# fbcotter/pytorch_wavelets

Measured on NVIDIA B200. Metric: Mpixels/sec DWT J=3 db4 + DTCWT J=3 fwd, higher is better.
Workload: dtype f32

## Files before the change

pytorch_wavelets_b200/csrc/b200wave.cu:

```cuda
#include <cuda_runtime.h>
#include <stdio.h>

#include "launch_params.h"
#include "fast_api.h"

namespace b200w {
constexpr int NT = 256;
extern __shared__ __align__(16) float g_smem[];

__global__ void __launch_bounds__(NT) k_afb2d_tile(const __grid_constant__ AfbParams p) { afb2d_tile<NT>(p, blockIdx.x, g_smem); }
__global__ void __launch_bounds__(NT) k_sfb2d_tile(const __grid_constant__ SfbParams p) { sfb2d_tile<NT>(p, blockIdx.x, g_smem); }
__global__ void __launch_bounds__(NT) k_fwd_j1_tile(const __grid_constant__ DtParams p) { fwd_j1_tile<NT, false>(p, blockIdx.x, g_smem); }
__global__ void __launch_bounds__(NT) k_scat_j1_tile(const __grid_constant__ DtParams p) { fwd_j1_tile<NT, true>(p, blockIdx.x, g_smem); }
__global__ void __launch_bounds__(NT) k_fwd_j2plus_tile(const __grid_constant__ DtParams p) { fwd_j2plus_tile<NT>(p, blockIdx.x, g_smem); }
__global__ void __launch_bounds__(NT) k_inv_j1_tile(const __grid_constant__ DtParams p) { inv_j1_tile<NT>(p, blockIdx.x, g_smem); }
__global__ void __launch_bounds__(NT) k_inv_j2plus_tile(const __grid_constant__ DtParams p) { inv_j2plus_tile<NT>(p, blockIdx.x, g_smem); }

}

using namespace b200w;

namespace {

thread_local char g_last_cuda_error[256] = "";

int check_launch() {
  cudaError_t e = cudaGetLastError();
  if (e != cudaSuccess) {
    snprintf(g_last_cuda_error, sizeof(g_last_cuda_error), "%s: %s", cudaGetErrorName(e), cudaGetErrorString(e));
    return B200W_ECUDA;
  }
  return B200W_OK;
}

template <class K>
int set_smem(K kernel, size_t bytes) {
  if (bytes > 48 * 1024) {
    if (bytes > 227 * 1024) return B200W_EFILTER;
    cudaError_t e = cudaFuncSetAttribute(kernel, cudaFuncAttributeMaxDynamicSharedMemorySize, (int)bytes);
    if (e != cudaSuccess) {
      snprintf(g_last_cuda_error, sizeof(g_last_cuda_error), "%s: %s", cudaGetErrorName(e), cudaGetErrorString(e));
      return B200W_ECUDA;
    }
  }
  return 0;
}

template <class K, class P>
int launch_tile(K kernel, const P& p, long long blocks, int smem_floats, void* stream) {
  if (blocks == 0) return B200W_OK;
  const size_t bytes = (size_t)smem_floats * sizeof(float);
  int rc = set_smem(kernel, bytes);
  if (rc) return rc;
  kernel<<<(unsigned)blocks, NT, bytes, (cudaStream_t)stream>>>(p);
  return check_launch();
}

}

namespace {

static int dwt_afb2d_impl(const float* x, long long x_plane_stride, int x_pitch, float* ll, long long ll_plane_stride,
                    int ll_pitch, float* highs, int planes, int H, int W, const float* fw_lo, const float* fw_hi,
                    int Lw, const float* fh_lo, const float* fh_hi, int Lh, int mode, void* stream, bool generic) {
  AfbParams p;
  int rc = build_afb(p, x, x_plane_stride, x_pitch, ll, ll_plane_stride, ll_pitch, highs, planes, H, W, fw_lo,
                     fw_hi, Lw, fh_lo, fh_hi, Lh, mode);
  if (rc) return rc;
  rc = generic ? fast::kNoFastPath : fast::try_launch_afb(p, (cudaStream_t)stream);
  if (rc != fast::kNoFastPath) return rc ? rc : check_launch();
  return launch_tile(k_afb2d_tile, p, (long long)planes * p.tiles_x * p.tiles_y, afb_smem_floats(Lw, Lh), stream);
}

static int dwt_sfb2d_impl(const float* ll, long long ll_plane_stride, int ll_pitch, const float* highs, float* y,
                    long long y_plane_stride, int y_pitch, int planes, int Hc, int Wc, int Ho, int Wo,
                    const float* gh_lo, const float* gh_hi, int Lh, const float* gw_lo, const float* gw_hi, int Lw,
                    int mode, void* stream, bool generic) {
  SfbParams p;
  int rc = build_sfb(p, ll, ll_plane_stride, ll_pitch, highs, y, y_plane_stride, y_pitch, planes, Hc, Wc, Ho, Wo,
                     gh_lo, gh_hi, Lh, gw_lo, gw_hi, Lw, mode);
  if (rc) return rc;
  rc = generic ? fast::kNoFastPath : fast::try_launch_sfb(p, (cudaStream_t)stream);
  if (rc != fast::kNoFastPath) return rc ? rc : check_launch();
  return launch_tile(k_sfb2d_tile, p, (long long)planes * p.tiles_x * p.tiles_y, sfb_smem_floats(Lh, Lw), stream);
}

static int dtcwt_fwd_j1_impl(const float* x, long long x_plane_stride, int x_pitch, float* ll, long long ll_plane_stride,
                       int ll_pitch, float* highs, const long long hs[6], int N, int C, int H, int W,
                       const float* h0, int L0, const float* h1, int L1, int mode, void* stream, bool generic) {
  DtParams p;
  int rc = build_fwd_j1(p, x, x_plane_stride, x_pitch, ll, ll_plane_stride, ll_pitch, highs, hs, N, C, H, W, h0, L0,
                        h1, L1, mode);
  if (rc) return rc;
  rc = generic ? fast::kNoFastPath : fast::try_launch_fwd_j1(p, (cudaStream_t)stream);
  if (rc != fast::kNoFastPath) return rc ? rc : check_launch();
  return launch_tile(k_fwd_j1_tile, p, (long long)N * C * p.tiles_x * p.tiles_y, fwdj1_smem_floats(L0, L1), stream);
}

static int dtcwt_fwd_j2plus_impl(const float* x, long long x_plane_stride, int x_pitch, float* ll,
                           long long ll_plane_stride, int ll_pitch, float* highs, const long long hs[6], int N,
                           int C, int H, int W, const float* h0a, const float* h1a, const float* h0b,
                           const float* h1b, int m, void* stream, bool generic) {
  DtParams p;
  int rc = build_fwd_j2plus(p, x, x_plane_stride, x_pitch, ll, ll_plane_stride, ll_pitch, highs, hs, N, C, H, W,
                            h0a, h1a, h0b, h1b, m);
  if (rc) return rc;
  rc = generic ? fast::kNoFastPath : fast::try_launch_fwd_j2plus(p, (cudaStream_t)stream);
  if (rc != fast::kNoFastPath) return rc ? rc : check_launch();
  return launch_tile(k_fwd_j2plus_tile, p, (long long)N * C * p.tiles_x * p.tiles_y, fwdj2_smem_floats(m), stream);
}

static int dtcwt_inv_j1_impl(const float* ll, long long ll_plane_stride, int ll_pitch, const float* highs,
                       const long long hs[6], float* y, long long y_plane_stride, int y_pitch, int N, int C, int H,
                       int W, const float* g0, int L0, const float* g1, int L1, int mode, void* stream, bool generic) {
  DtParams p;
  int rc = build_inv_j1(p, ll, ll_plane_stride, ll_pitch, highs, hs, y, y_plane_stride, y_pitch, N, C, H, W, g0, L0,
                        g1, L1, mode);
  if (rc) return rc;
  rc = generic ? fast::kNoFastPath : fast::try_launch_inv_j1(p, (cudaStream_t)stream);
  if (rc != fast::kNoFastPath) return rc ? rc : check_launch();
  return launch_tile(k_inv_j1_tile, p, (long long)N * C * p.tiles_x * p.tiles_y, invj1_smem_floats(L0, L1), stream);
}

static int dtcwt_inv_j2plus_impl(const float* ll, long long ll_plane_stride, int ll_pitch, const float* highs,
                           const long long hs[6], float* y, long long y_plane_stride, int y_pitch, int N, int C,
                           int H, int W, const float* g0a, const float* g1a, const float* g0b, const float* g1b,
                           int m, void* stream, bool generic) {
  DtParams p;
  int rc = build_inv_j2plus(p, ll, ll_plane_stride, ll_pitch, highs, hs, y, y_plane_stride, y_pitch, N, C, H, W,
                            g0a, g1a, g0b, g1b, m);
  if (rc) return rc;
  rc = generic ? fast::kNoFastPath : fast::try_launch_inv_j2plus(p, (cudaStream_t)stream);
  if (rc != fast::kNoFastPath) return rc ? rc : check_launch();
  return launch_tile(k_inv_j2plus_tile, p, (long long)N * C * p.tiles_x * p.tiles_y, invj2_smem_floats(m), stream);
}

static int scat_j1_impl(const float* x, float* z, float* dre_dr, float* dim_dr, int N, int C, int H, int W,
                  const float* h0, int L0, const float* h1, int L1, int mode, float magbias, void* stream, bool generic) {
  DtParams p;
  int rc = build_scat_j1(p, x, z, dre_dr, dim_dr, N, C, H, W, h0, L0, h1, L1, mode, magbias);
  if (rc) return rc;
  rc = generic ? fast::kNoFastPath : fast::try_launch_scat_j1(p, (cudaStream_t)stream);
  if (rc != fast::kNoFastPath) return rc ? rc : check_launch();
  return launch_tile(k_scat_j1_tile, p, (long long)N * C * p.tiles_x * p.tiles_y, fwdj1_smem_floats(L0, L1), stream);
}

}

extern "C" {

int b200w_version(void) { return B200W_VERSION; }

const char* b200w_strerror(int code) {
  switch (code) {
    case B200W_OK: return "ok";
    case B200W_EMODE: return "Unkown pad type";
    case B200W_ESIZE: return "bad tensor size";
    case B200W_EARG: return "bad argument";
    case B200W_EFILTER: return "unsupported filter length";
    case B200W_ECUDA: return "CUDA error";
    case B200W_ENOTIMPL: return "not implemented";
    default: return "unknown error";
  }
}

const char* b200w_last_cuda_error(void) { return g_last_cuda_error; }

int b200w_dwt_coeff_len(int n, int flen, int mode) { return coeff_len(n, flen, mode); }
int b200w_dwt_rec_len(int k, int flen, int mode) { return rec_len(k, flen, mode); }

int b200w_dwt_afb2d(const float* x, long long x_plane_stride, int x_pitch, float* ll, long long ll_plane_stride,
                    int ll_pitch, float* highs, int planes, int H, int W, const float* fw_lo, const float* fw_hi,
                    int Lw, const float* fh_lo, const float* fh_hi, int Lh, int mode, void* stream) {
  return dwt_afb2d_impl(x, x_plane_stride, x_pitch, ll, ll_plane_stride, ll_pitch, highs, planes, H, W, fw_lo, fw_hi, Lw, fh_lo, fh_hi, Lh, mode, stream, false);
}
int b200w_dwt_afb2d_generic(const float* x, long long x_plane_stride, int x_pitch, float* ll, long long ll_plane_stride,
                    int ll_pitch, float* highs, int planes, int H, int W, const float* fw_lo, const float* fw_hi,
                    int Lw, const float* fh_lo, const float* fh_hi, int Lh, int mode, void* stream) {
  return dwt_afb2d_impl(x, x_plane_stride, x_pitch, ll, ll_plane_stride, ll_pitch, highs, planes, H, W, fw_lo, fw_hi, Lw, fh_lo, fh_hi, Lh, mode, stream, true);
}

int b200w_dwt_sfb2d(const float* ll, long long ll_plane_stride, int ll_pitch, const float* highs, float* y,
                    long long y_plane_stride, int y_pitch, int planes, int Hc, int Wc, int Ho, int Wo,
                    const float* gh_lo, const float* gh_hi, int Lh, const float* gw_lo, const float* gw_hi, int Lw,
                    int mode, void* stream) {
  return dwt_sfb2d_impl(ll, ll_plane_stride, ll_pitch, highs, y, y_plane_stride, y_pitch, planes, Hc, Wc, Ho, Wo, gh_lo, gh_hi, Lh, gw_lo, gw_hi, Lw, mode, stream, false);
}
int b200w_dwt_sfb2d_generic(const float* ll, long long ll_plane_stride, int ll_pitch, const float* highs, float* y,
                    long long y_plane_stride, int y_pitch, int planes, int Hc, int Wc, int Ho, int Wo,
                    const float* gh_lo, const float* gh_hi, int Lh, const float* gw_lo, const float* gw_hi, int Lw,
                    int mode, void* stream) {
  return dwt_sfb2d_impl(ll, ll_plane_stride, ll_pitch, highs, y, y_plane_stride, y_pitch, planes, Hc, Wc, Ho, Wo, gh_lo, gh_hi, Lh, gw_lo, gw_hi, Lw, mode, stream, true);
}

int b200w_dtcwt_fwd_j1(const float* x, long long x_plane_stride, int x_pitch, float* ll, long long ll_plane_stride,
                       int ll_pitch, float* highs, const long long hs[6], int N, int C, int H, int W,
                       const float* h0, int L0, const float* h1, int L1, int mode, void* stream) {
  return dtcwt_fwd_j1_impl(x, x_plane_stride, x_pitch, ll, ll_plane_stride, ll_pitch, highs, hs, N, C, H, W, h0, L0, h1, L1, mode, stream, false);
}
int b200w_dtcwt_fwd_j1_generic(const float* x, long long x_plane_stride, int x_pitch, float* ll, long long ll_plane_stride,
                       int ll_pitch, float* highs, const long long hs[6], int N, int C, int H, int W,
                       const float* h0, int L0, const float* h1, int L1, int mode, void* stream) {
  return dtcwt_fwd_j1_impl(x, x_plane_stride, x_pitch, ll, ll_plane_stride, ll_pitch, highs, hs, N, C, H, W, h0, L0, h1, L1, mode, stream, true);
}

int b200w_dtcwt_fwd_j2plus(const float* x, long long x_plane_stride, int x_pitch, float* ll,
                           long long ll_plane_stride, int ll_pitch, float* highs, const long long hs[6], int N,
                           int C, int H, int W, const float* h0a, const float* h1a, const float* h0b,
                           const float* h1b, int m, void* stream) {
  return dtcwt_fwd_j2plus_impl(x, x_plane_stride, x_pitch, ll, ll_plane_stride, ll_pitch, highs, hs, N, C, H, W, h0a, h1a, h0b, h1b, m, stream, false);
}
int b200w_dtcwt_fwd_j2plus_generic(const float* x, long long x_plane_stride, int x_pitch, float* ll,
                           long long ll_plane_stride, int ll_pitch, float* highs, const long long hs[6], int N,
                           int C, int H, int W, const float* h0a, const float* h1a, const float* h0b,
                           const float* h1b, int m, void* stream) {
  return dtcwt_fwd_j2plus_impl(x, x_plane_stride, x_pitch, ll, ll_plane_stride, ll_pitch, highs, hs, N, C, H, W, h0a, h1a, h0b, h1b, m, stream, true);
}

int b200w_dtcwt_inv_j1(const float* ll, long long ll_plane_stride, int ll_pitch, const float* highs,
                       const long long hs[6], float* y, long long y_plane_stride, int y_pitch, int N, int C, int H,
                       int W, const float* g0, int L0, const float* g1, int L1, int mode, void* stream) {
  return dtcwt_inv_j1_impl(ll, ll_plane_stride, ll_pitch, highs, hs, y, y_plane_stride, y_pitch, N, C, H, W, g0, L0, g1, L1, mode, stream, false);
}
int b200w_dtcwt_inv_j1_generic(const float* ll, long long ll_plane_stride, int ll_pitch, const float* highs,
                       const long long hs[6], float* y, long long y_plane_stride, int y_pitch, int N, int C, int H,
                       int W, const float* g0, int L0, const float* g1, int L1, int mode, void* stream) {
  return dtcwt_inv_j1_impl(ll, ll_plane_stride, ll_pitch, highs, hs, y, y_plane_stride, y_pitch, N, C, H, W, g0, L0, g1, L1, mode, stream, true);
}

int b200w_dtcwt_inv_j2plus(const float* ll, long long ll_plane_stride, int ll_pitch, const float* highs,
                           const long long hs[6], float* y, long long y_plane_stride, int y_pitch, int N, int C,
                           int H, int W, const float* g0a, const float* g1a, const float* g0b, const float* g1b,
                           int m, void* stream) {
  return dtcwt_inv_j2plus_impl(ll, ll_plane_stride, ll_pitch, highs, hs, y, y_plane_stride, y_pitch, N, C, H, W, g0a, g1a, g0b, g1b, m, stream, false);
}
int b200w_dtcwt_inv_j2plus_generic(const float* ll, long long ll_plane_stride, int ll_pitch, const float* highs,
                           const long long hs[6], float* y, long long y_plane_stride, int y_pitch, int N, int C,
                           int H, int W, const float* g0a, const float* g1a, const float* g0b, const float* g1b,
                           int m, void* stream) {
  return dtcwt_inv_j2plus_impl(ll, ll_plane_stride, ll_pitch, highs, hs, y, y_plane_stride, y_pitch, N, C, H, W, g0a, g1a, g0b, g1b, m, stream, true);
}


static long long align256(long long n) { return (n + 255) / 256 * 256; }

static void dwt_ws_layout(int planes, int H, int W, int J, int Lw, int Lh, int mode, long long bytes[2]) {
  bytes[0] = bytes[1] = 0;
  int h = H, w = W;
  for (int j = 0; j + 1 < J; ++j) {
    h = coeff_len(h, Lh, mode); w = coeff_len(w, Lw, mode);
    if (h < 1 || w < 1) break;
    const long long need = align256(4LL * planes * h * ((w + 31) / 32 * 32));
    if (need > bytes[j & 1]) bytes[j & 1] = need;
  }
}

enum DwtPolicy { kLevels = 0, kPyramidFirst = 1, kPyramidAll = 2 };

#ifndef B200W_PYR_FUSE_ALL_MIN_WIDTH
#define B200W_PYR_FUSE_ALL_MIN_WIDTH 1024
#endif

static DwtPolicy dwt_policy(PyrParams& pp, const float* x, long long xps, int xpitch, int planes, int H, int W, int J,
                            int Lw, int Lh, int mode, bool generic) {
  if (generic || Lw != Lh) return kLevels;
  const bool wide = (W >= B200W_PYR_FUSE_ALL_MIN_WIDTH);
  if ((J == 1 || wide) && fast::plan_dwt_pyramid(pp, x, xps, xpitch, planes, H, W, J, Lw, mode, 0) == 0)
    return kPyramidAll;
  if (J >= 2) {
    const int wo = coeff_len(W, Lw, mode);
    if (wo > 0 && fast::plan_dwt_pyramid(pp, x, xps, xpitch, planes, H, W, 1, Lw, mode, (wo + 31) / 32 * 32) == 0)
      return kPyramidFirst;
  }
  return kLevels;
}

long long b200w_dwt_forward_workspace(const float* x, long long x_plane_stride, int x_pitch, int planes, int H, int W,
                                      int J, int Lw, int Lh, int mode) {
  if (!dwt_mode_ok(mode)) return B200W_EMODE;
  if (planes < 0 || H < 1 || W < 1 || J < 1) return B200W_ESIZE;
  if (Lw < 2 || Lh < 2 || Lw > kMaxTaps || Lh > kMaxTaps) return B200W_EFILTER;
  PyrParams pp;
  if (dwt_policy(pp, x, x_plane_stride, x_pitch, planes, H, W, J, Lw, Lh, mode, false) == kPyramidAll) return 0;
  long long b[2];
  dwt_ws_layout(planes, H, W, J, Lw, Lh, mode, b);
  return b[0] + b[1];
}

static void pyr_set_taps(PyrParams& pp, const float* fw_lo, const float* fw_hi, const float* fh_lo, const float* fh_hi,
                         int L) {
  for (int i = 0; i < kPyrMaxTaps; ++i) {
    const bool on = i < L;
    pp.fw[2 * i] = on ? fw_lo[i] : 0.f; pp.fw[2 * i + 1] = on ? fw_hi[i] : 0.f;
    pp.fh_lo[i] = on ? fh_lo[i] : 0.f; pp.fh_hi[i] = on ? fh_hi[i] : 0.f;
  }
}

static int dwt_forward_impl(const float* x, long long x_plane_stride, int x_pitch, int planes, int H, int W, int J,
                            float* yl, float* const* highs, const float* fw_lo, const float* fw_hi, int Lw,
                            const float* fh_lo, const float* fh_hi, int Lh, int mode, void* workspace,
                            long long workspace_bytes, void* stream, bool generic) {
  if (!dwt_mode_ok(mode)) return B200W_EMODE;
  if (!x || !yl || !highs || !fw_lo || !fw_hi || !fh_lo || !fh_hi) return B200W_EARG;
  if (planes < 0 || H < 1 || W < 1 || J < 1) return B200W_ESIZE;
  if (Lw < 2 || Lh < 2) return B200W_EFILTER;
  for (int j = 0; j < J; ++j)
    if (!highs[j]) return B200W_EARG;
  PyrParams pp;
  DwtPolicy pol = dwt_policy(pp, x, x_plane_stride, x_pitch, planes, H, W, J, Lw, Lh, mode, generic);
  if (pol == kPyramidAll) {
    pyr_set_taps(pp, fw_lo, fw_hi, fh_lo, fh_hi, Lw);
    pp.yl = yl;
    for (int j = 0; j < kPyrMaxLevels; ++j) pp.highs[j] = (j < J) ? highs[j] : nullptr;
    const int rc = fast::launch_dwt_pyramid(pp, (cudaStream_t)stream);
    if (rc != fast::kNoFastPath) return rc ? rc : check_launch();
    pol = kLevels;
  }
  long long wb[2];
  dwt_ws_layout(planes, H, W, J, Lw, Lh, mode, wb);
  if (wb[0] + wb[1] > 0 && (!workspace || workspace_bytes < wb[0] + wb[1])) return B200W_EARG;
  float* buf[2] = {static_cast<float*>(workspace), reinterpret_cast<float*>(static_cast<char*>(workspace) + wb[0])};
  const float* src = x;
  long long sps = x_plane_stride;
  int spitch = x_pitch, h = H, w = W;
  for (int j = 0; j < J; ++j) {
    const int ho = coeff_len(h, Lh, mode), wo = coeff_len(w, Lw, mode);
    if (ho < 1 || wo < 1) return B200W_ESIZE;
    const bool last = (j == J - 1);
    const int wp = last ? wo : (wo + 31) / 32 * 32;
    float* ll = last ? yl : buf[j & 1];
    int rc = fast::kNoFastPath;
    if (j == 0 && pol == kPyramidFirst) {
      pyr_set_taps(pp, fw_lo, fw_hi, fh_lo, fh_hi, Lw);
      pp.yl = ll;
      for (int i = 0; i < kPyrMaxLevels; ++i) pp.highs[i] = (i == 0) ? highs[0] : nullptr;
      rc = fast::launch_dwt_pyramid(pp, (cudaStream_t)stream);
      if (rc == 0) rc = check_launch();
    }
    if (rc == fast::kNoFastPath)
      rc = dwt_afb2d_impl(src, sps, spitch, ll, (long long)ho * wp, wp, highs[j], planes, h, w, fw_lo, fw_hi, Lw, fh_lo,
                          fh_hi, Lh, mode, stream, generic);
    if (rc) return rc;
    src = ll; sps = (long long)ho * wp; spitch = wp; h = ho; w = wo;
  }
  return B200W_OK;
}

int b200w_dwt_forward(const float* x, long long x_plane_stride, int x_pitch, int planes, int H, int W, int J, float* yl,
                      float* const* highs, const float* fw_lo, const float* fw_hi, int Lw, const float* fh_lo,
                      const float* fh_hi, int Lh, int mode, void* workspace, long long workspace_bytes, void* stream) {
  return dwt_forward_impl(x, x_plane_stride, x_pitch, planes, H, W, J, yl, highs, fw_lo, fw_hi, Lw, fh_lo, fh_hi, Lh,
                          mode, workspace, workspace_bytes, stream, false);
}
int b200w_dwt_forward_generic(const float* x, long long x_plane_stride, int x_pitch, int planes, int H, int W, int J,
                              float* yl, float* const* highs, const float* fw_lo, const float* fw_hi, int Lw,
                              const float* fh_lo, const float* fh_hi, int Lh, int mode, void* workspace,
                              long long workspace_bytes, void* stream) {
  return dwt_forward_impl(x, x_plane_stride, x_pitch, planes, H, W, J, yl, highs, fw_lo, fw_hi, Lw, fh_lo, fh_hi, Lh,
                          mode, workspace, workspace_bytes, stream, true);
}

int b200w_scat_j1(const float* x, float* z, float* dre_dr, float* dim_dr, int N, int C, int H, int W,
                  const float* h0, int L0, const float* h1, int L1, int mode, float magbias, void* stream) {
  return scat_j1_impl(x, z, dre_dr, dim_dr, N, C, H, W, h0, L0, h1, L1, mode, magbias, stream, false);
}
int b200w_scat_j1_generic(const float* x, float* z, float* dre_dr, float* dim_dr, int N, int C, int H, int W,
                  const float* h0, int L0, const float* h1, int L1, int mode, float magbias, void* stream) {
  return scat_j1_impl(x, z, dre_dr, dim_dr, N, C, H, W, h0, L0, h1, L1, mode, magbias, stream, true);
}

}
```

pytorch_wavelets_b200/csrc/dwt_pyramid.cuh:

```cuda
#pragma once
#include "pyramid_plan.h"
#include "stream_common.cuh"

namespace b200w {
namespace fast {

#ifdef B200W_PYR_PROF
__device__ unsigned long long g_pyr_prof[64];
#define PYR_T0() const long long pyr_t0_ = clock64()
#define PYR_ACC(k) prof[k] += (unsigned long long)(clock64() - pyr_t0_)
#define PYR_DECL() unsigned long long prof[8] = {0, 0, 0, 0, 0, 0, 0, 0}; const long long pyr_life_ = clock64()
#define PYR_FLUSH(role, lane)                                                                              \
  do {                                                                                                     \
    prof[7] = (unsigned long long)(clock64() - pyr_life_);                                                 \
    if ((lane) == 0)                                                                                       \
      for (int k_ = 0; k_ < 8; ++k_) atomicAdd(&g_pyr_prof[8 * (role) + k_], prof[k_]);                    \
  } while (0)
#else
#define PYR_T0() do {} while (0)
#define PYR_ACC(k) do {} while (0)
#define PYR_DECL() do {} while (0)
#define PYR_FLUSH(role, lane) do {} while (0)
#endif

constexpr int kPyrNSlotC = B200W_PYR_NSLOT;

template <int L>
struct PyrCfg {
  static constexpr int NC = kPyrNC;
  static constexpr int PL = L - 2;
  static constexpr int PRO = PL / 2;
  static constexpr int UNR = L / 2;
  static constexpr int HS = pyr_hs(L);
  static constexpr int RS = 2 * HS;
  static constexpr int HALO = pyr_halo(L);
  static constexpr int NX = 2 * NC + PL;
  static_assert(HS >= 4 && HS % 2 == 0 && HS % UNR == 0, "stage = whole window periods, even");
};

__device__ __forceinline__ void mbar_arrive(unsigned bar) {
  asm volatile("mbarrier.arrive.shared::cta.b64 _, [%0];\n" ::"r"(bar) : "memory");
}
__device__ __forceinline__ bool mbar_test(unsigned bar, unsigned parity) {
  unsigned ok;
  asm volatile(
      "{\n.reg .pred p;\n"
      "mbarrier.test_wait.parity.shared::cta.b64 p, [%1], %2;\n"
      "selp.u32 %0, 1, 0, p;\n}\n"
      : "=r"(ok)
      : "r"(bar), "r"(parity)
      : "memory");
  return ok != 0;
}
__device__ __forceinline__ void mbar_wait_relaxed(unsigned bar, unsigned parity) {
  while (!mbar_test(bar, parity)) __nanosleep(200);
}
__device__ __forceinline__ void bulk_store_s2g(float* gdst, unsigned ssrc, unsigned bytes) {
  asm volatile("cp.async.bulk.global.shared::cta.bulk_group [%0], [%1], %2;\n" ::"l"(gdst), "r"(ssrc), "r"(bytes) : "memory");
}
__device__ __forceinline__ void bulk_commit() { asm volatile("cp.async.bulk.commit_group;\n" ::: "memory"); }
template <int N>
__device__ __forceinline__ void bulk_wait_read() { asm volatile("cp.async.bulk.wait_group.read %0;\n" ::"n"(N) : "memory"); }
template <int N>
__device__ __forceinline__ void bulk_wait() { asm volatile("cp.async.bulk.wait_group %0;\n" ::"n"(N) : "memory"); }
__device__ __forceinline__ void bulk_load_g2s(unsigned sdst, const float* gsrc, unsigned bytes, unsigned bar) {
  asm volatile("cp.async.bulk.shared::cluster.global.mbarrier::complete_tx::bytes [%0], [%1], %2, [%3];\n" ::"r"(sdst),
               "l"(gsrc), "r"(bytes), "r"(bar)
               : "memory");
}

__device__ __forceinline__ int pyr_phase(const float* band_base) {
  return (int)((reinterpret_cast<uintptr_t>(band_base) >> 2) & 3);
}
__device__ __forceinline__ float* pyr_band_base(const PyrParams& p, int l, int b, int plane) {
  const PyrLevel& v = p.lv[l];
  const long long band = (long long)v.Ho * v.Wo;
  if (b == 3) return p.yl + (long long)plane * v.Ho * p.ll_pitch;
  return p.highs[l] + ((long long)plane * 3 + b) * band;
}

template <int L>
__device__ __forceinline__ void pyr_producer(const PyrParams& p, int plane, float* smem, unsigned bar0, int lane) {
  using C = PyrCfg<L>;
  const PyrLevel& v = p.lv[0];
  const float* src_plane = p.x + (long long)plane * p.xps;
  const int n_slots = 2 * v.n_stage;
  const unsigned row_bytes = (unsigned)v.W * 4u;
  float* ring = smem + v.in_off;
  const unsigned ring_s = (unsigned)__cvta_generic_to_shared(ring);
  PYR_DECL();
#pragma unroll 1
  for (int q = 0; q < n_slots; ++q) {
    const int slot = q % kPyrNSlotC;
    const int use = q / kPyrNSlotC;
    if (use > 0) { PYR_T0(); mbar_wait(bar0 + 8 * (v.bar_in + v.n_in + slot), (unsigned)((use - 1) & 1)); PYR_ACC(0); }
    int src = -1;
    if (lane < C::HS) src = ext_index(q * C::HS + lane - C::PL, v.H, p.mode);
    const unsigned valid = __ballot_sync(0xffffffffu, src >= 0);
    unsigned zero_rows = ((1u << C::HS) - 1u) & ~valid;
    while (zero_rows) {
      const int j = __ffs(zero_rows) - 1;
      zero_rows &= zero_rows - 1;
      float* dst = ring + (slot * C::HS + j) * v.in_pitch + C::HALO;
      for (int i = lane * 4; i < v.W; i += 128) *reinterpret_cast<float4*>(dst + i) = make_float4(0.f, 0.f, 0.f, 0.f);
    }
    __syncwarp();
    const unsigned full = bar0 + 8 * (v.bar_in + slot);
    if (lane == 0) mbar_arrive_expect_tx(full, (unsigned)__popc(valid) * row_bytes);
    __syncwarp();
    if (src >= 0)
      bulk_load_g2s(ring_s + 4u * (unsigned)((slot * C::HS + lane) * v.in_pitch + C::HALO),
                    src_plane + (long long)src * p.xpitch, row_bytes, full);
  }
  PYR_FLUSH(0, lane);
}

template <int L, int SPLIT>
__device__ __forceinline__ void pyr_writer(const PyrParams& p, int plane, float* smem, unsigned bar0, int lane) {
  using C = PyrCfg<L>;
  const int SG = C::HS / SPLIT;
  const int R = kPyrNGO * SG;
  const bool bulk_lane = lane < 4;
  const int myb = bulk_lane ? lane : (lane >= 8 ? (lane - 8) / 6 : 4);
  const int mye = (lane >= 8) ? (lane - 8) % 6 : 0;
  float* gb[kPyrMaxLevels];
  unsigned stb[kPyrMaxLevels];
  int ph[kPyrMaxLevels], next_g[kPyrMaxLevels], rslot[kPyrMaxLevels];
  int remaining = 0;
#pragma unroll
  for (int l = 0; l < kPyrMaxLevels; ++l) {
    next_g[l] = 0; rslot[l] = 0; gb[l] = nullptr; stb[l] = 0; ph[l] = 0;
    if (l < p.J) {
      remaining += p.lv[l].n_stage * SPLIT;
      if (myb < p.lv[l].nbands) {
        gb[l] = pyr_band_base(p, l, myb, plane);
        ph[l] = pyr_phase(gb[l]);
        stb[l] = (unsigned)__cvta_generic_to_shared(smem) + 4u * (unsigned)(p.lv[l].st_off + myb * p.lv[l].st_cap);
      }
    }
  }
  int prev_bar = -1;
  PYR_DECL();

  while (remaining > 0) {
    bool any = false;
#pragma unroll
    for (int l = 0; l < kPyrMaxLevels; ++l) {
      if (l >= p.J) break;
      const PyrLevel& v = p.lv[l];
      const int g = next_g[l];
      if (g >= v.n_stage * SPLIT) continue;
      const int bar = v.bar_out + g % kPyrNGO;
      if (!__all_sync(0xffffffffu, mbar_test(bar0 + 8 * bar, (unsigned)((g / kPyrNGO) & 1)))) continue;
      any = true;
      PYR_T0();
      const int k0 = imax(0, g * SG - C::PRO), k1 = imin(v.Ho, (g + 1) * SG - C::PRO);
      if (k1 > k0 && gb[l] != nullptr) {
        const int rowlen = (myb == 3) ? p.ll_pitch : v.Wo;
        const int cap = (myb == 3) ? v.st_cap_ll : v.st_cap;
        const int s0 = k0 * rowlen, s1 = k1 * rowlen, a = ph[l];
        const int hd = imin(s1 - s0, (4 - ((s0 + a) & 3)) & 3);
        const int m0 = s0 + hd;
        const int m1 = m0 + ((s1 - m0) & ~3);
        int i0 = rslot[l] * rowlen + a;
        if (bulk_lane) {
          const int n = m1 - m0;
          if (n > 0) {
            int i = i0 + hd;
            if (i >= cap) i -= cap;
            const int first = imin(n, cap - i);
            bulk_store_s2g(gb[l] + m0, stb[l] + 4u * (unsigned)i, 4u * (unsigned)first);
            if (n > first) bulk_store_s2g(gb[l] + m0 + first, stb[l], 4u * (unsigned)(n - first));
          }
        } else {
          int pos = -1;
          if (mye < 3) { if (mye < hd) pos = s0 + mye; }
          else if (mye - 3 < s1 - m1) pos = m1 + (mye - 3);
          if (pos >= 0) {
            int i = i0 + (pos - s0);
            while (i >= cap) i -= cap;
            gb[l][pos] = lds_s(stb[l] + 4u * (unsigned)i);
          }
        }
      }
      if (k1 > k0) { rslot[l] += k1 - k0; if (rslot[l] >= R) rslot[l] -= R; }
      bulk_commit();
      bulk_wait_read<1>();
      __syncwarp();
      if (prev_bar >= 0 && lane == 0) mbar_arrive(bar0 + 8 * prev_bar);
      prev_bar = bar + kPyrNGO;
      next_g[l] = g + 1;
      --remaining;
      PYR_ACC(0);
#ifdef B200W_PYR_PROF
      prof[1] += 1;
#endif
    }
    if (!any) {
      if (prev_bar >= 0) {
        PYR_T0();
        bulk_wait_read<0>();
        PYR_ACC(2);
        __syncwarp();
        if (lane == 0) mbar_arrive(bar0 + 8 * prev_bar);
        prev_bar = -1;
      } else {
        __nanosleep(100);
      }
    }
  }
  { PYR_T0(); bulk_wait<0>(); PYR_ACC(3); }
  PYR_FLUSH(1, lane);
}

__device__ __forceinline__ float2 lds64_s(unsigned s) {
  float2 v;
  asm volatile("ld.shared.v2.f32 {%0, %1}, [%2];\n" : "=f"(v.x), "=f"(v.y) : "r"(s));
  return v;
}
template <int OFF>
__device__ __forceinline__ float2 lds64_so(unsigned s) {
  float2 v;
  asm volatile("ld.shared.v2.f32 {%0, %1}, [%2+%3];\n" : "=f"(v.x), "=f"(v.y) : "r"(s), "n"(OFF));
  return v;
}
template <int OFF>
__device__ __forceinline__ void sts_so(unsigned s, float v) {
  asm volatile("st.shared.f32 [%0+%2], %1;\n" ::"r"(s), "f"(v), "n"(OFF) : "memory");
}
__device__ __forceinline__ uint2 lds64u_s(unsigned s) {
  uint2 v;
  asm volatile("ld.shared.v2.u32 {%0, %1}, [%2];\n" : "=r"(v.x), "=r"(v.y) : "r"(s));
  return v;
}
__device__ __forceinline__ void stsu_s(unsigned s, unsigned v) { asm volatile("st.shared.u32 [%0], %1;\n" ::"r"(s), "r"(v) : "memory"); }

template <int L>
__device__ __forceinline__ void pyr_rowpass(const PyrParams& p, unsigned row_s, float2 (&dst)[PyrCfg<L>::NC]) {
  using C = PyrCfg<L>;
  float x[C::NX];
  {
    float2 v;
#define PYR_LD(Q) if constexpr (Q < C::NX / 2) { v = lds64_so<8 * (Q)>(row_s); x[2 * (Q)] = v.x; x[2 * (Q) + 1] = v.y; }
    PYR_LD(0) PYR_LD(1) PYR_LD(2) PYR_LD(3) PYR_LD(4) PYR_LD(5) PYR_LD(6) PYR_LD(7) PYR_LD(8) PYR_LD(9) PYR_LD(10) PYR_LD(11)
#undef PYR_LD
    static_assert(C::NX / 2 <= 12, "unrolled loads");
  }
#pragma unroll
  for (int o = 0; o < C::NC; ++o) {
    float2 r = make_float2(0.f, 0.f);
#pragma unroll
    for (int j = 0; j < L; ++j) r = ffma2_s(x[2 * o + j], make_float2(p.fw[2 * j], p.fw[2 * j + 1]), r);
    dst[o] = r;
  }
}

template <int L>
struct PyrEmit {
  unsigned st_s[4];
  unsigned so[4];
  unsigned capb, wob;
  unsigned capb3, wob3;
  int nv, nb, kslot, R;
  unsigned nr_s;
  unsigned nr_off, nr_pitch4, nr_bytes;
  int dup[kPyrNC];

  __device__ __forceinline__ void putn(int b, const float (&v)[kPyrNC], bool wrap_slot) {
    const unsigned a = st_s[b] + so[b];
    if (!wrap_slot) {
      if (nv > 0) sts_so<0>(a, v[0]);
      if (nv > 1) sts_so<4>(a, v[1]);
      if constexpr (kPyrNC > 2) { if (nv > 2) sts_so<8>(a, v[kPyrNC > 2 ? 2 : 0]); }
    } else {
#pragma unroll
      for (int i = 0; i < kPyrNC; ++i) {
        const unsigned cb = (b == 3) ? capb3 : capb;
        unsigned oi = so[b] + 4u * i;
        if (oi >= cb) oi -= cb;
        if (nv > i) sts_s(st_s[b] + oi, v[i]);
      }
    }
  }
  __device__ __forceinline__ void row(const float2 (&lo)[kPyrNC], const float2 (&hi)[kPyrNC]) {
    float v0[kPyrNC], v1[kPyrNC], v2[kPyrNC], v3[kPyrNC];
#pragma unroll
    for (int i = 0; i < kPyrNC; ++i) { v0[i] = hi[i].x; v1[i] = lo[i].y; v2[i] = hi[i].y; v3[i] = lo[i].x; }
    const bool wrap_slot = (kslot == R - 1);
    putn(0, v0, wrap_slot);
    putn(1, v1, wrap_slot);
    putn(2, v2, wrap_slot);
    if (nb == 4) putn(3, v3, wrap_slot);
#pragma unroll
    for (int b = 0; b < 3; ++b) so[b] = so[b] + wob - (wrap_slot ? capb : 0u);
    so[3] = so[3] + wob3 - (wrap_slot ? capb3 : 0u);
    kslot = wrap_slot ? 0 : kslot + 1;
    if (nr_s != 0) {
      const unsigned rb = nr_s + nr_off;
      if (nv > 0) sts_so<0>(rb, v3[0]);
      if (nv > 1) sts_so<4>(rb, v3[1]);
      if constexpr (kPyrNC > 2) { if (nv > 2) sts_so<8>(rb, v3[kPyrNC > 2 ? 2 : 0]); }
#pragma unroll
      for (int i = 0; i < kPyrNC; ++i)
        if (dup[i] != 0) sts_s(rb + 4u * i + (unsigned)dup[i], v3[i]);
      nr_off += nr_pitch4;
      if (nr_off >= nr_bytes) nr_off = 0;
    }
  }
};

template <int L, int SPLIT>
__device__ __forceinline__ void pyr_worker(const PyrParams& p, int plane, int lvl, int wl, int warp, int lane,
                                           float* smem, unsigned bar0) {
  using C = PyrCfg<L>;
  const PyrLevel& v = p.lv[lvl];
  const bool last = (lvl == p.J - 1);
  const int c0 = C::NC * (32 * wl + lane);
  const int nv = imax(0, imin(C::NC, v.Wo - c0));
  const unsigned rd4 = 4u * (unsigned)((nv > 0) ? (C::HALO + 2 * c0 - C::PL) : C::HALO);
  const unsigned smem_s = (unsigned)__cvta_generic_to_shared(smem);
  const unsigned ring_s = smem_s + 4u * (unsigned)v.in_off;
  const unsigned zero_s = smem_s + 4u * (unsigned)p.zero_off;
  const unsigned tab_s = smem_s + 4u * (unsigned)(p.tab_off + 32 * warp);

  PyrEmit<L> em;
  em.capb = 4u * (unsigned)v.st_cap; em.wob = 4u * (unsigned)v.Wo; em.nv = nv; em.nb = v.nbands;
  em.capb3 = 4u * (unsigned)v.st_cap_ll; em.wob3 = 4u * (unsigned)p.ll_pitch;
  em.kslot = 0; em.R = kPyrNGO * (C::HS / SPLIT);
#pragma unroll
  for (int b = 0; b < 4; ++b) {
    em.st_s[b] = smem_s + 4u * (unsigned)(v.st_off + (b < v.nbands ? b : 0) * v.st_cap);
    em.so[b] = (b < v.nbands) ? 4u * (unsigned)(c0 + pyr_phase(pyr_band_base(p, lvl, b, plane))) : 0u;
  }
  em.nr_s = 0; em.nr_off = 0; em.nr_pitch4 = 0; em.nr_bytes = 1;
#pragma unroll
  for (int i = 0; i < C::NC; ++i) em.dup[i] = 0;
  int nx_bar = 0, nx_n = 1;
  if (!last) {
    const PyrLevel& u = p.lv[lvl + 1];
    em.nr_s = smem_s + 4u * (unsigned)(u.in_off + C::HALO + c0);
    em.nr_pitch4 = 4u * (unsigned)u.in_pitch;
    em.nr_bytes = em.nr_pitch4 * (unsigned)u.in_rows;
    nx_bar = u.bar_in; nx_n = u.n_in;
    const int Wn = v.Wo;
#pragma unroll
    for (int i = 0; i < C::NC; ++i) {
      const int c = c0 + i;
      int cell = c;
      if (i < nv) {
        if (p.mode == B200W_MODE_SYMMETRIC) {
          if (c < C::PL) cell = -1 - c;
          else if (c >= Wn - (L - 1)) cell = 2 * Wn - 1 - c;
        } else if (p.mode == B200W_MODE_REFLECT) {
          if (c >= 1 && c <= C::PL) cell = -c;
          else if (c <= Wn - 2 && c >= Wn - L) cell = 2 * Wn - 2 - c;
        }
      }
      em.dup[i] = 4 * (cell - c);
    }
  }
  const int cw0 = C::NC * 32 * wl, cw1 = imin(cw0 + C::NC * 32, v.Wo);
  const bool patch_l = (lvl == 0) && (p.mode != B200W_MODE_ZERO) && (2 * cw0 - C::PL < 0);
  const bool patch_r = (lvl == 0) && (p.mode != B200W_MODE_ZERO) && (2 * (cw1 - 1) + 1 >= v.W);
  int patch_dst = -1, patch_src = 0;
  if (patch_l && lane < C::PL) {
    const int j = lane + 1;
    patch_dst = C::HALO - j;
    patch_src = C::HALO + ((p.mode == B200W_MODE_SYMMETRIC) ? j - 1 : j);
  } else if (patch_r && lane >= C::PL && lane < C::PL + L - 1) {
    const int i = lane - C::PL;
    patch_dst = C::HALO + v.W + i;
    patch_src = C::HALO + ((p.mode == B200W_MODE_SYMMETRIC) ? v.W - 1 - i : v.W - 2 - i);
  }
  const bool do_patch = patch_l || patch_r;

  float2 w[L][C::NC];
#pragma unroll
  for (int j = 0; j < L; ++j)
#pragma unroll
    for (int o = 0; o < C::NC; ++o) w[j][o] = make_float2(0.f, 0.f);

  PYR_DECL();
  int g_seen = 0, g_rel = 0;
  const int prev_stages = (lvl > 0) ? p.lv[lvl - 1].n_stage : 0;
  const int pitch4 = 4 * v.in_pitch;
  constexpr int split = SPLIT, nslot = kPyrNSlotC;

#pragma unroll 1
  for (int t = 0; t < v.n_stage; ++t) {
    if (lane < C::RS) {
      unsigned a;
      if (lvl == 0) {
        const int slot = (2 * t + (lane >= C::HS ? 1 : 0)) % nslot;
        a = ring_s + (unsigned)((slot * C::HS + (lane >= C::HS ? lane - C::HS : lane)) * pitch4);
      } else {
        const int e = t * C::RS + lane - C::PL;
        const int src = ((unsigned)e < (unsigned)v.H) ? e : ext_index_cold(e, v.H, p.mode);
        a = (src >= 0) ? ring_s + (unsigned)((src % v.in_rows) * pitch4) : zero_s;
      }
      stsu_s(tab_s + 4u * lane, a);
    }
    if (!last && t >= nx_n) { PYR_T0(); mbar_wait(bar0 + 8 * (nx_bar + nx_n + t % nx_n), (unsigned)((t / nx_n - 1) & 1)); PYR_ACC(2); }
    if (lvl > 0) {
      const int g_need = imin(pyr_group_of_row(pyr_stage_max_row(t, C::RS, C::PL, v.H, p.mode), C::HS, C::PRO),
                              prev_stages - 1);
      PYR_T0();
      while (g_seen <= g_need) {
        mbar_wait_relaxed(bar0 + 8 * (v.bar_in + g_seen % v.n_in), (unsigned)((g_seen / v.n_in) & 1));
        ++g_seen;
      }
      PYR_ACC(0);
    }
    __syncwarp();
    const int k_first = t * C::HS - C::PRO;
#pragma unroll
    for (int hh = 0; hh < C::HS; ++hh) {
      if (hh == 0 || (split == 2 && hh == C::HS / 2)) {
        const int sg = t * split + (hh ? 1 : 0);
        if (sg >= kPyrNGO) {
          PYR_T0();
          mbar_wait(bar0 + 8 * (v.bar_out + kPyrNGO + sg % kPyrNGO), (unsigned)((sg / kPyrNGO - 1) & 1));
          PYR_ACC(1);
        }
      }
      if (lvl == 0 && (hh == 0 || hh == C::HS / 2)) {
        const int q = 2 * t + (hh ? 1 : 0);
        if (hh) {
          __syncwarp();
          if (lane == 0) mbar_arrive(bar0 + 8 * (v.bar_in + v.n_in + (q - 1) % nslot));
        }
        const int slot = q % nslot;
        { PYR_T0(); mbar_wait(bar0 + 8 * (v.bar_in + slot), (unsigned)((q / nslot) & 1)); PYR_ACC(0); }
        if (do_patch) {
          PYR_T0();
          if (patch_dst >= 0) {
            const unsigned a = ring_s + (unsigned)(slot * C::HS * pitch4);
#pragma unroll
            for (int j = 0; j < C::HS; ++j)
              sts_s(a + (unsigned)(j * pitch4 + 4 * patch_dst), lds_s(a + (unsigned)(j * pitch4 + 4 * patch_src)));
          }
          __syncwarp();
          PYR_ACC(4);
        }
      }
      const uint2 ra = lds64u_s(tab_s + 8u * hh);
      pyr_rowpass<L>(p, ra.x + rd4, w[(2 * hh) % L]);
      pyr_rowpass<L>(p, ra.y + rd4, w[(2 * hh + 1) % L]);
      const int k = k_first + hh;
      if (k >= 0 && k < v.Ho) {
        PYR_T0();
        float2 lo[C::NC], hi[C::NC];
#pragma unroll
        for (int o = 0; o < C::NC; ++o) {
          float2 a0 = make_float2(0.f, 0.f), a1 = make_float2(0.f, 0.f);
#pragma unroll
          for (int j = 0; j < L; ++j) {
            a0 = ffma2_s(p.fh_lo[j], w[(2 * hh + 2 + j) % L][o], a0);
            a1 = ffma2_s(p.fh_hi[j], w[(2 * hh + 2 + j) % L][o], a1);
          }
          lo[o] = a0; hi[o] = a1;
        }
        em.row(lo, hi);
        PYR_ACC(5);
      }
      if (split == 2 && hh == C::HS / 2 - 1) {
        fence_proxy_async();
        __syncwarp();
        if (lane == 0) mbar_arrive(bar0 + 8 * (v.bar_out + (t * split) % kPyrNGO));
      }
    }
#ifdef B200W_PYR_PROF
    const long long pyr_tf_ = clock64();
#endif
    fence_proxy_async();
    __syncwarp();
#ifdef B200W_PYR_PROF
    prof[3] += (unsigned long long)(clock64() - pyr_tf_);
#endif
    if (lane == 0) {
      if (lvl == 0) mbar_arrive(bar0 + 8 * (v.bar_in + v.n_in + (2 * t + 1) % nslot));
      mbar_arrive(bar0 + 8 * (v.bar_out + (t * split + split - 1) % kPyrNGO));
      if (!last) mbar_arrive(bar0 + 8 * (nx_bar + t % nx_n));
    }
    if (lvl > 0) {
      const int lo_row = pyr_stage_release_bound(t, C::RS, C::PL, v.H, L);
      while (g_rel < prev_stages && pyr_group_end(g_rel, C::HS, C::PRO) <= lo_row) {
        if (lane == 0) mbar_arrive(bar0 + 8 * (v.bar_in + v.n_in + g_rel % v.n_in));
        ++g_rel;
      }
    }
  }
  PYR_FLUSH(2 + lvl, lane);
}

template <int L, int MAXT, int MINB, int SPLIT>
__global__ void __launch_bounds__(MAXT, MINB) dwt_pyramid(const __grid_constant__ PyrParams p) {
  extern __shared__ __align__(128) float smem[];
  const int tid = threadIdx.x, warp = tid >> 5, lane = tid & 31;
  const int plane = blockIdx.x;
  const unsigned bar0 = (unsigned)__cvta_generic_to_shared(smem);

  {
    const int n4 = p.smem_bytes / 16;
    float4* s4 = reinterpret_cast<float4*>(smem);
    for (int i = tid; i < n4; i += blockDim.x) s4[i] = make_float4(0.f, 0.f, 0.f, 0.f);
  }
  __syncthreads();
  if (tid == 0) {
    for (int l = 0; l < p.J; ++l) {
      const PyrLevel& v = p.lv[l];
      const int n_up = (l == 0) ? 1 : p.lv[l - 1].nwarps;
      for (int i = 0; i < v.n_in; ++i) {
        mbar_init(bar0 + 8 * (v.bar_in + i), (unsigned)n_up);
        mbar_init(bar0 + 8 * (v.bar_in + v.n_in + i), (unsigned)v.nwarps);
      }
      for (int i = 0; i < kPyrNGO; ++i) {
        mbar_init(bar0 + 8 * (v.bar_out + i), (unsigned)v.nwarps);
        mbar_init(bar0 + 8 * (v.bar_out + kPyrNGO + i), 1u);
      }
    }
    mbar_fence_init();
  }
  fence_proxy_async();
  __syncthreads();

  if (warp == 0) {
    pyr_producer<L>(p, plane, smem, bar0, lane);
  } else if (warp == 1) {
    pyr_writer<L, SPLIT>(p, plane, smem, bar0, lane);
  } else {
    int lvl = 0;
#pragma unroll
    for (int l = 1; l < kPyrMaxLevels; ++l)
      if (l < p.J && warp >= p.lv[l].warp0) lvl = l;
    pyr_worker<L, SPLIT>(p, plane, lvl, warp - p.lv[lvl].warp0, warp, lane, smem, bar0);
  }
}

template <int L, int MAXT, int MINB, int SPLIT>
inline int launch_pyramid_v(const PyrParams& p, cudaStream_t stream, int slot) {
  static int smem_set[64] = {};
  int dev = 0;
  (void)cudaGetDevice(&dev);
  (void)slot;
  if (dev < 0 || dev >= 64 || !smem_set[dev]) {
    if (cudaFuncSetAttribute(dwt_pyramid<L, MAXT, MINB, SPLIT>, cudaFuncAttributeMaxDynamicSharedMemorySize, 227 * 1024) != cudaSuccess) {
      (void)cudaGetLastError();
      return kNoFastPath;
    }
    if (dev >= 0 && dev < 64) smem_set[dev] = 1;
  }
  dwt_pyramid<L, MAXT, MINB, SPLIT><<<(unsigned)p.planes, p.threads, p.smem_bytes, stream>>>(p);
  return 0;
}

template <int L>
inline int launch_pyramid(const PyrParams& p, cudaStream_t stream) {
  if (p.planes <= 0) return 0;
  if (p.threads <= 160) {
    if (p.split != pyr_split(L)) return kNoFastPath;
    return launch_pyramid_v<L, 160, pyr_minb_small(L), pyr_split(L)>(p, stream, 0);
  }
  if (p.split != 1) return kNoFastPath;
  if (p.threads <= 256) return launch_pyramid_v<L, 256, 2, 1>(p, stream, 1);
  return launch_pyramid_v<L, 512, 1, 1>(p, stream, 2);
}

}
}
```

pytorch_wavelets_b200/csrc/fast_api.h:

```cpp
#pragma once
#include <cuda_runtime.h>

#include "common.h"
#include "pyramid_plan.h"

namespace b200w {
namespace fast {

constexpr int kNoFastPath = 1;

int try_launch_afb(const AfbParams& p, cudaStream_t stream);
int try_launch_sfb(const SfbParams& p, cudaStream_t stream);
int try_launch_fwd_j1(const DtParams& p, cudaStream_t stream);
int try_launch_scat_j1(const DtParams& p, cudaStream_t stream);
int try_launch_fwd_j2plus(const DtParams& p, cudaStream_t stream);
int try_launch_inv_j1(const DtParams& p, cudaStream_t stream);
int try_launch_inv_j2plus(const DtParams& p, cudaStream_t stream);

int plan_dwt_pyramid(PyrParams& p, const float* x, long long xps, int xpitch, int planes, int H, int W, int J, int L,
                     int mode, int ll_pitch);
int launch_dwt_pyramid(const PyrParams& p, cudaStream_t stream);

}
}
```

pytorch_wavelets_b200/csrc/k_pyramid.cu:

```cuda
#include "dwt_pyramid.cuh"

namespace b200w {
namespace fast {

static int max_optin_smem() {
  static int cache[64] = {};
  int dev = 0;
  if (cudaGetDevice(&dev) != cudaSuccess || dev < 0 || dev >= 64) return 227 * 1024;
  if (cache[dev] == 0) {
    int v = 0;
    if (cudaDeviceGetAttribute(&v, cudaDevAttrMaxSharedMemoryPerBlockOptin, dev) != cudaSuccess || v <= 0) {
      (void)cudaGetLastError();
      v = 227 * 1024;
    }
    cache[dev] = v;
  }
  return cache[dev];
}

static int sm_smem() {
  static int cache[64] = {};
  int dev = 0;
  if (cudaGetDevice(&dev) != cudaSuccess || dev < 0 || dev >= 64) return 228 * 1024;
  if (cache[dev] == 0) {
    int v = 0;
    if (cudaDeviceGetAttribute(&v, cudaDevAttrMaxSharedMemoryPerMultiprocessor, dev) != cudaSuccess || v <= 0) {
      (void)cudaGetLastError();
      v = 228 * 1024;
    }
    cache[dev] = v;
  }
  return cache[dev];
}

int plan_dwt_pyramid(PyrParams& p, const float* x, long long xps, int xpitch, int planes, int H, int W, int J, int L,
                     int mode, int ll_pitch) {
  return plan_pyramid_best(p, planes, H, W, J, L, mode, xps, xpitch, x, max_optin_smem(), sm_smem(), ll_pitch)
             ? kNoFastPath : 0;
}

int launch_dwt_pyramid(const PyrParams& p, cudaStream_t stream) {
  switch (p.L) {
    case 2: return launch_pyramid<2>(p, stream);
    case 4: return launch_pyramid<4>(p, stream);
    case 6: return launch_pyramid<6>(p, stream);
    case 8: return launch_pyramid<8>(p, stream);
    case 10: return launch_pyramid<10>(p, stream);
    case 12: return launch_pyramid<12>(p, stream);
    default: return kNoFastPath;
  }
}

}
}

#ifdef B200W_PYR_PROF
extern "C" int b200w_debug_pyr_prof(unsigned long long* out) {
  unsigned long long z[64] = {};
  if (cudaDeviceSynchronize() != cudaSuccess) return -1;
  if (cudaMemcpyFromSymbol(out, b200w::fast::g_pyr_prof, sizeof(z)) != cudaSuccess) return -2;
  if (cudaMemcpyToSymbol(b200w::fast::g_pyr_prof, z, sizeof(z)) != cudaSuccess) return -3;
  return 0;
}
#endif
```

pytorch_wavelets_b200/csrc/pyramid_plan.h:

```cpp
#pragma once
#include "common.h"

namespace b200w {

constexpr int kPyrMaxLevels = 4;
constexpr int kPyrMaxTaps = 16;
#ifndef B200W_PYR_NC
#define B200W_PYR_NC 3
#endif
constexpr int kPyrNC = B200W_PYR_NC;
constexpr int kPyrNGO = 2;
#ifndef B200W_PYR_SPLIT
#define B200W_PYR_SPLIT 2
#endif
#ifndef B200W_PYR_NSLOT
#define B200W_PYR_NSLOT 4
#endif
constexpr int kPyrAuxWarps = 2;

struct PyrLevel {
  int H, W, Ho, Wo;
  int n_stage;
  int warp0, nwarps;
  int in_off, in_pitch, in_rows;
  int n_in;
  int bar_in;
  int st_off, st_cap, nbands;
  int st_cap_ll;
  int bar_out;
};

struct PyrParams {
  const float* x; long long xps; int xpitch;
  float* yl;
  float* highs[kPyrMaxLevels];
  int planes, J, mode, L;
  int nslot;
  int split;
  int ll_pitch;
  int zero_off;
  int tab_off;
  int n_bars, smem_bytes, threads;
  PyrLevel lv[kPyrMaxLevels];
  alignas(16) float fw[2 * kPyrMaxTaps];
  alignas(16) float fh_lo[kPyrMaxTaps];
  alignas(16) float fh_hi[kPyrMaxTaps];
};

constexpr int pyr_hs(int L) {
  int m = 1;
  while ((L / 2) * m < 4 || (((L / 2) * m) & 1)) ++m;
  return (L / 2) * m;
}
constexpr int pyr_halo(int L) { return (L - 2 + 3) / 4 * 4; }
constexpr int pyr_split(int L) { return (pyr_hs(L) % 4 == 0) ? B200W_PYR_SPLIT : 1; }

B200W_HD int pyr_group_end(int g, int HS, int PRO) { return (g + 1) * HS - PRO; }
B200W_HD int pyr_group_of_row(int r, int HS, int PRO) { return (r + PRO) / HS; }

B200W_HD int pyr_stage_max_row(int t, int RS, int PL, int H, int mode) {
  const int e0 = t * RS - PL, e1 = e0 + RS - 1;
  int hi = imin(e1, H - 1);
  if (e0 < 0) {
    const int g = ext_index(e0, H, mode);
    if (g > hi) hi = g;
  }
  if (hi < 0) hi = 0;
  return hi;
}
B200W_HD int pyr_stage_release_bound(int t, int RS, int PL, int H, int L) {
  return imin((t + 1) * RS - PL, H - L + 1);
}

inline int plan_pyramid(PyrParams& p, int planes, int H, int W, int J, int L, int mode, long long xps, int xpitch,
                        const void* x, int max_smem_bytes, int nslot = 4, int split = 1, int extra_in = 1,
                        int ll_pitch = 0) {
  if (J < 1 || J > kPyrMaxLevels) return 1;
  if (L < 2 || (L & 1) || L > 12) return 1;
  if (mode != B200W_MODE_ZERO && mode != B200W_MODE_SYMMETRIC && mode != B200W_MODE_REFLECT) return 1;
  if ((W & 3) || (xpitch & 3) || (xps & 3) || (reinterpret_cast<uintptr_t>(x) & 15)) return 1;
  const int HS = pyr_hs(L), RS = 2 * HS, PL = L - 2, PRO = PL / 2, HALO = pyr_halo(L);
  p.planes = planes; p.J = J; p.mode = mode; p.L = L;
  p.nslot = nslot; p.split = split;
  if (nslot < 3 || nslot > 4 || (split != 1 && split != 2) || (HS % split)) return 1;
  int warp = kPyrAuxWarps;
  int h = H, w = W;
  int nbar = 0;
  int off = 0;
  for (int l = 0; l < J; ++l) {
    PyrLevel& v = p.lv[l];
    if (h < L || w < L) return 1;
    if (l > 0 && w < 2 * L - 2) return 1;
    v.H = h; v.W = w;
    v.Ho = (h + L - 1) / 2; v.Wo = (w + L - 1) / 2;
    v.n_stage = (v.Ho + PRO + HS - 1) / HS;
    const int lanes = (v.Wo + kPyrNC - 1) / kPyrNC;
    v.nwarps = (lanes + 31) / 32;
    v.warp0 = warp; warp += v.nwarps;
    v.in_pitch = (HALO + 2 * (v.Wo + kPyrNC - 2) + 2 + 3) / 4 * 4;
    if (v.in_pitch < HALO + w + L - 1) v.in_pitch = (HALO + w + L - 1 + 3) / 4 * 4;
    if (l == 0) {
      v.n_in = nslot;
      v.in_rows = nslot * HS;
    } else {
      const PyrLevel& u = p.lv[l - 1];
      int need = 1, rel = 0;
      for (int t = 0; t < v.n_stage; ++t) {
        const int g_need = imin(pyr_group_of_row(pyr_stage_max_row(t, RS, PL, h, mode), HS, PRO), u.n_stage - 1);
        if (g_need - rel + 1 > need) need = g_need - rel + 1;
        const int lo = pyr_stage_release_bound(t, RS, PL, h, L);
        while (rel < u.n_stage && pyr_group_end(rel, HS, PRO) <= lo) ++rel;
      }
      v.n_in = need + extra_in;
      v.in_rows = v.n_in * HS;
    }
    v.in_off = off; off += v.in_rows * v.in_pitch;
    v.bar_in = nbar; nbar += 2 * v.n_in;
    v.nbands = (l == J - 1) ? 4 : 3;
    v.st_cap = kPyrNGO * (HS / split) * v.Wo;
    v.st_cap_ll = 0;
    if (l == J - 1) {
      p.ll_pitch = (ll_pitch > 0) ? ll_pitch : v.Wo;
      if (p.ll_pitch < v.Wo) return 1;
      v.st_cap_ll = kPyrNGO * (HS / split) * p.ll_pitch;
    }
    if ((v.st_cap & 3) || (v.st_cap_ll & 3)) return 1;
    v.st_off = off; off += 3 * v.st_cap + v.st_cap_ll;
    v.bar_out = nbar; nbar += 2 * kPyrNGO;
    h = v.Ho; w = v.Wo;
  }
  int maxpitch = 0;
  for (int l = 0; l < J; ++l) maxpitch = imax(maxpitch, p.lv[l].in_pitch);
  p.zero_off = off; off += (maxpitch + 2 * kPyrNC + 8 + 3) / 4 * 4;
  p.tab_off = off; off += 32 * warp;
  p.n_bars = nbar;
  const int bar_floats = (2 * nbar + 31) / 32 * 32;
  for (int l = 0; l < J; ++l) { p.lv[l].in_off += bar_floats; p.lv[l].st_off += bar_floats; }
  p.zero_off += bar_floats;
  p.tab_off += bar_floats;
  p.smem_bytes = (off + bar_floats) * 4;
  p.threads = 32 * warp;
  if (p.threads > 512 || p.smem_bytes > max_smem_bytes) return 1;
  p.x = static_cast<const float*>(x); p.xps = xps; p.xpitch = xpitch;
  return 0;
}

#ifndef B200W_PYR_MINB_SMALL
#define B200W_PYR_MINB_SMALL 4
#endif
constexpr int pyr_minb_small(int L) { return (L <= 8) ? B200W_PYR_MINB_SMALL : (B200W_PYR_MINB_SMALL < 3 ? B200W_PYR_MINB_SMALL : 3); }
inline int pyr_ctas_for_threads(int threads, int L) { return threads <= 160 ? pyr_minb_small(L) : (threads <= 256 ? 2 : 1); }

inline int plan_pyramid_best(PyrParams& p, int planes, int H, int W, int J, int L, int mode, long long xps, int xpitch,
                             const void* x, int max_smem_bytes, int sm_smem_bytes, int ll_pitch = 0) {
  PyrParams best;
  int best_ctas = 0;
  for (int split = 1; split <= 2; ++split) {
    PyrParams q;
    if (plan_pyramid(q, planes, H, W, J, L, mode, xps, xpitch, x, max_smem_bytes, B200W_PYR_NSLOT, split, 1, ll_pitch))
      continue;
    if (split != ((q.threads <= 160) ? pyr_split(L) : 1)) continue;
    const int by_smem = sm_smem_bytes / (q.smem_bytes + 1024);
    const int ctas = imin(by_smem, pyr_ctas_for_threads(q.threads, L));
    if (ctas > best_ctas) { best_ctas = ctas; best = q; }
  }
  if (best_ctas == 0) return 1;
  p = best;
  return 0;
}

}
```

Measured before the change: 375,500.

## Fuse remaining DWT levels into one pyramid kernel after first level

```diff
diff --git a/pytorch_wavelets_b200/csrc/b200wave.cu b/pytorch_wavelets_b200/csrc/b200wave.cu
--- a/pytorch_wavelets_b200/csrc/b200wave.cu
+++ b/pytorch_wavelets_b200/csrc/b200wave.cu
@@ -256,6 +256,10 @@
 }
 
 enum DwtPolicy { kLevels = 0, kPyramidFirst = 1, kPyramidAll = 2 };
+
+#ifndef B200W_PYR_REST_MIN_WIDTH
+#define B200W_PYR_REST_MIN_WIDTH 256
+#endif
 
 #ifndef B200W_PYR_FUSE_ALL_MIN_WIDTH
 #define B200W_PYR_FUSE_ALL_MIN_WIDTH 1024
@@ -324,6 +328,16 @@
   long long sps = x_plane_stride;
   int spitch = x_pitch, h = H, w = W;
   for (int j = 0; j < J; ++j) {
+    if (j == 1 && pol == kPyramidFirst && J >= 3 && w >= B200W_PYR_REST_MIN_WIDTH) {
+      PyrParams pr;
+      if (fast::plan_dwt_pyramid(pr, src, sps, spitch, planes, h, w, J - 1, Lw, mode, 0, true) == 0 && pr.threads <= 160) {
+        pyr_set_taps(pr, fw_lo, fw_hi, fh_lo, fh_hi, Lw);
+        pr.yl = yl;
+        for (int i = 0; i < kPyrMaxLevels; ++i) pr.highs[i] = (i < J - 1) ? highs[i + 1] : nullptr;
+        const int rc = fast::launch_dwt_pyramid(pr, (cudaStream_t)stream);
+        if (rc != fast::kNoFastPath) return rc ? rc : check_launch();
+      }
+    }
     const int ho = coeff_len(h, Lh, mode), wo = coeff_len(w, Lw, mode);
     if (ho < 1 || wo < 1) return B200W_ESIZE;
     const bool last = (j == J - 1);
diff --git a/pytorch_wavelets_b200/csrc/dwt_pyramid.cuh b/pytorch_wavelets_b200/csrc/dwt_pyramid.cuh
--- a/pytorch_wavelets_b200/csrc/dwt_pyramid.cuh
+++ b/pytorch_wavelets_b200/csrc/dwt_pyramid.cuh
@@ -85,7 +85,7 @@
   const PyrLevel& v = p.lv[0];
   const float* src_plane = p.x + (long long)plane * p.xps;
   const int n_slots = 2 * v.n_stage;
-  const unsigned row_bytes = (unsigned)v.W * 4u;
+  const unsigned row_bytes = (unsigned)pyr_row_floats(v.W) * 4u;
   float* ring = smem + v.in_off;
   const unsigned ring_s = (unsigned)__cvta_generic_to_shared(ring);
   PYR_DECL();
diff --git a/pytorch_wavelets_b200/csrc/fast_api.h b/pytorch_wavelets_b200/csrc/fast_api.h
--- a/pytorch_wavelets_b200/csrc/fast_api.h
+++ b/pytorch_wavelets_b200/csrc/fast_api.h
@@ -18,7 +18,7 @@
 int try_launch_inv_j2plus(const DtParams& p, cudaStream_t stream);
 
 int plan_dwt_pyramid(PyrParams& p, const float* x, long long xps, int xpitch, int planes, int H, int W, int J, int L,
-                     int mode, int ll_pitch);
+                     int mode, int ll_pitch, bool pad_readable = false);
 int launch_dwt_pyramid(const PyrParams& p, cudaStream_t stream);
 
 }
diff --git a/pytorch_wavelets_b200/csrc/k_pyramid.cu b/pytorch_wavelets_b200/csrc/k_pyramid.cu
--- a/pytorch_wavelets_b200/csrc/k_pyramid.cu
+++ b/pytorch_wavelets_b200/csrc/k_pyramid.cu
@@ -34,8 +34,9 @@
 }
 
 int plan_dwt_pyramid(PyrParams& p, const float* x, long long xps, int xpitch, int planes, int H, int W, int J, int L,
-                     int mode, int ll_pitch) {
-  return plan_pyramid_best(p, planes, H, W, J, L, mode, xps, xpitch, x, max_optin_smem(), sm_smem(), ll_pitch)
+                     int mode, int ll_pitch, bool pad_readable) {
+  return plan_pyramid_best(p, planes, H, W, J, L, mode, xps, xpitch, x, max_optin_smem(), sm_smem(), ll_pitch,
+                           pad_readable)
              ? kNoFastPath : 0;
 }
 
diff --git a/pytorch_wavelets_b200/csrc/pyramid_plan.h b/pytorch_wavelets_b200/csrc/pyramid_plan.h
--- a/pytorch_wavelets_b200/csrc/pyramid_plan.h
+++ b/pytorch_wavelets_b200/csrc/pyramid_plan.h
@@ -53,6 +53,7 @@
   return (L / 2) * m;
 }
 constexpr int pyr_halo(int L) { return (L - 2 + 3) / 4 * 4; }
+B200W_HD int pyr_row_floats(int W) { return (W + 3) & ~3; }
 constexpr int pyr_split(int L) { return (pyr_hs(L) % 4 == 0) ? B200W_PYR_SPLIT : 1; }
 
 B200W_HD int pyr_group_end(int g, int HS, int PRO) { return (g + 1) * HS - PRO; }
@@ -74,11 +75,12 @@
 
 inline int plan_pyramid(PyrParams& p, int planes, int H, int W, int J, int L, int mode, long long xps, int xpitch,
                         const void* x, int max_smem_bytes, int nslot = 4, int split = 1, int extra_in = 1,
-                        int ll_pitch = 0) {
+                        int ll_pitch = 0, bool pad_readable = false) {
   if (J < 1 || J > kPyrMaxLevels) return 1;
   if (L < 2 || (L & 1) || L > 12) return 1;
   if (mode != B200W_MODE_ZERO && mode != B200W_MODE_SYMMETRIC && mode != B200W_MODE_REFLECT) return 1;
-  if ((W & 3) || (xpitch & 3) || (xps & 3) || (reinterpret_cast<uintptr_t>(x) & 15)) return 1;
+  if ((xpitch & 3) || (xps & 3) || (reinterpret_cast<uintptr_t>(x) & 15)) return 1;
+  if ((W & 3) && (!pad_readable || mode == B200W_MODE_ZERO || xpitch < pyr_row_floats(W))) return 1;
   const int HS = pyr_hs(L), RS = 2 * HS, PL = L - 2, PRO = PL / 2, HALO = pyr_halo(L);
   p.planes = planes; p.J = J; p.mode = mode; p.L = L;
   p.nslot = nslot; p.split = split;
@@ -152,12 +154,14 @@
 inline int pyr_ctas_for_threads(int threads, int L) { return threads <= 160 ? pyr_minb_small(L) : (threads <= 256 ? 2 : 1); }
 
 inline int plan_pyramid_best(PyrParams& p, int planes, int H, int W, int J, int L, int mode, long long xps, int xpitch,
-                             const void* x, int max_smem_bytes, int sm_smem_bytes, int ll_pitch = 0) {
+                             const void* x, int max_smem_bytes, int sm_smem_bytes, int ll_pitch = 0,
+                             bool pad_readable = false) {
   PyrParams best;
   int best_ctas = 0;
   for (int split = 1; split <= 2; ++split) {
     PyrParams q;
-    if (plan_pyramid(q, planes, H, W, J, L, mode, xps, xpitch, x, max_smem_bytes, B200W_PYR_NSLOT, split, 1, ll_pitch))
+    if (plan_pyramid(q, planes, H, W, J, L, mode, xps, xpitch, x, max_smem_bytes, B200W_PYR_NSLOT, split, 1, ll_pitch,
+                     pad_readable))
       continue;
     if (split != ((q.threads <= 160) ? pyr_split(L) : 1)) continue;
     const int by_smem = sm_smem_bytes / (q.smem_bytes + 1024);
```

After: 344,300, median of 6. 0.917x the previous value.
